# martende/findex

Measured on NVIDIA B200. Metric: fm_count_queries_per_s_len16_1GB_text, higher is better.
Workload: dtype u32

## Files before the change

### findex_b200/csrc/fmx_device.cuh

```cuda
#pragma once
#include <cstdint>
#include <cuda_runtime.h>

#include "../../include/fmgpu.h"

namespace fmx {

constexpr uint32_t kBitsPerBlock = 480;
constexpr int kCodeAbsent = 0xFF;

struct DevIndex {
    const uint4   *blocks;
    uint64_t       stride;
    const uint8_t *bwt;
    const uint32_t *C;
    const uint32_t *base;
    const uint8_t *code;
    const uint4   *mark;
    const uint32_t *samples;
    const uint4   *bm;
    uint32_t n, eof;
    int32_t  layout, levels;
    uint32_t z[8];
    int32_t  wmx_b, wmx_levels;
// ... 375 lines not shown
        if (stop) return false;
        base += G;
        if (base >= ix.dict_buckets) base = 0;
        first = false;
    }
    return false;
}

template <int G, bool STATS, bool BISECT, typename PatFn>
__device__ __forceinline__ bool dict_chain(const DevIndex &ix, const uint8_t *code, PatFn pat, int &i, uint32_t &sp, uint32_t &ep,
                                           uint32_t &touched, uint32_t &steps, int depth, bool top_known_missed = false) {
    const int Jc = ix.dict_Jc;
    const uint32_t bits = (uint32_t)ix.dict_bits;
    for (int t = (depth - ix.dict_D) / Jc + 1; t <= kDictMaxTiers && i >= 0 && depth < ix.dict_Dx; ++t) {
        const int j = (i + 1) < Jc ? (i + 1) : Jc;
        uint64_t syms = 0;
        bool ok = true;
        for (int k = 0; k < j; ++k) {
            const uint32_t c = pat(i - k), cd = code[c];
            ok = ok && (cd != (uint32_t)kCodeAbsent) && (c != 0);
            syms |= (uint64_t)cd << (bits * (uint32_t)k);
        }
        if (!ok) return true;
        uint32_t s, e;
        if (!top_known_missed && dict_probe<G, STATS>(ix, dict_chain_key(sp, j, t, syms), s, e, touched)) {
            sp = s; ep = e;
            i -= j;
            depth += j;
            if (STATS) steps += j;
            if (j < Jc) return true;
            continue;
        }
        if (!BISECT) return false;
        int lo = 0, hi = j - 1;
        uint32_t bs = 0, be = 0;
        const uint32_t psp = sp;
        while (lo < hi) {
            const int mid = (lo + hi + 1) >> 1;
            if (dict_probe<G, STATS>(ix, dict_chain_key(psp, mid, t, syms & ((1ull << (bits * (uint32_t)mid)) - 1ull)), s, e, touched)) { lo = mid; bs = s; be = e; }
            else hi = mid - 1;
        }
        if (lo > 0) { sp = bs; ep = be; i -= lo; if (STATS) steps += lo; }
        return true;
    }
    return true;
}

struct CtxQuery {
    unsigned long long qlo, qhi, mlo, mhi;
    uint32_t sh;
    bool zero, absent;
};
template <typename PatFn>
__device__ __forceinline__ CtxQuery ctx_query(const DevIndex &ix, const SharedTables &tb, PatFn pat, int j, int o) {
    CtxQuery q;
    const uint32_t bits = (uint32_t)ix.isat_bits;
    q.qlo = 0; q.qhi = 0;
    q.sh = (uint32_t)(ix.ctx_J - j) * bits;
    const uint32_t nb = (uint32_t)j * bits;
    q.mlo = nb >= 64 ? ~0ull : ((1ull << nb) - 1ull);
    q.mhi = nb <= 64 ? 0ull : ((1ull << (nb - 64)) - 1ull);
    q.zero = false; q.absent = false;
    if (ix.ctx_raw) {
        uint32_t w0, w1, w2;
        pat.bytes12(o, w0, w1, w2);
        q.qlo = ((unsigned long long)w1 << 32) | w0;
        q.qhi = w2;
        const unsigned long long l = q.qlo | ~q.mlo, h = (q.qhi & q.mhi) | ~q.mhi;
        q.zero = (((l - 0x0101010101010101ull) & ~l) | ((h - 0x0101010101010101ull) & ~h)) & 0x8080808080808080ull;
    } else {
        for (int k = 0; k < j; ++k) {
            const uint32_t pc = pat(o + k), cd = tb.code[pc];
            q.zero = q.zero || (pc == 0);
            q.absent = q.absent || (cd == (uint32_t)kCodeAbsent);
            const unsigned long long v = (unsigned long long)((cd + 1u) & ((1u << bits) - 1u));
            const uint32_t ob = (uint32_t)k * bits;
            if (ob < 64) { q.qlo |= v << ob; if (ob + bits > 64) q.qhi |= v >> (64 - ob); }
            else q.qhi |= v << (ob - 64);
        }
    }
    return q;
}
__device__ __forceinline__ bool ctx_match(const CtxQuery &q, const uint4 &b) {
    const unsigned long long elo = ((unsigned long long)b.z << 32) | b.y, ehi = b.w;
    unsigned long long lo, hi;
    if (q.sh == 0) { lo = elo; hi = ehi; }
    else if (q.sh < 64) { lo = (elo >> q.sh) | (ehi << (64 - q.sh)); hi = ehi >> q.sh; }
    else { lo = ehi >> (q.sh - 64); hi = 0; }
    return (((lo ^ q.qlo) & q.mlo) | ((hi ^ q.qhi) & q.mhi)) == 0ull;
}

constexpr uint32_t kKmerGroup = 8, kKmerWide = 0xFFu, kKmerInlineRows = 3;

template <int G, bool STATS, typename PatFn>
__device__ __forceinline__ void kmer_group(const DevIndex &ix, const SharedTables &tb, PatFn pat, bool fetch, uint32_t idx, int &i,
                                           uint32_t &sp, uint32_t &ep, uint32_t &touched, uint32_t &steps, uint32_t &pre_from,
                                           uint32_t &pre_best, uint32_t &pre_cnt) {
    const uint4 *blk = reinterpret_cast<const uint4 *>(ix.kmer) + (uint64_t)(idx / kKmerGroup) * 4;
    uint4 q0, q1, q2, q3;
    if constexpr (G == 1) {
        const uint32_t odd = threadIdx.x & 1u;
        const unsigned long long mine = reinterpret_cast<unsigned long long>(blk);
        const unsigned long long pe = __shfl_sync(0xFFFFFFFFu, mine, (threadIdx.x & 31u) & ~1u);
        const unsigned long long po = __shfl_sync(0xFFFFFFFFu, mine, (threadIdx.x & 31u) | 1u);
        const bool fe = __shfl_sync(0xFFFFFFFFu, fetch, (threadIdx.x & 31u) & ~1u), fo = __shfl_sync(0xFFFFFFFFu, fetch, (threadIdx.x & 31u) | 1u);
        uint4 x0 = make_uint4(0, 0, 0, 0), x1 = x0, y0 = x0, y1 = x0;
        if (fe) ldg256(reinterpret_cast<const uint4 *>(pe) + 2 * odd, x0, x1);
        if (fo) ldg256(reinterpret_cast<const uint4 *>(po) + 2 * odd, y0, y1);
        uint4 s0 = odd ? x0 : y0, s1 = odd ? x1 : y1;
        s0.x = __shfl_xor_sync(0xFFFFFFFFu, s0.x, 1); s0.y = __shfl_xor_sync(0xFFFFFFFFu, s0.y, 1);
        s0.z = __shfl_xor_sync(0xFFFFFFFFu, s0.z, 1); s0.w = __shfl_xor_sync(0xFFFFFFFFu, s0.w, 1);
        s1.x = __shfl_xor_sync(0xFFFFFFFFu, s1.x, 1); s1.y = __shfl_xor_sync(0xFFFFFFFFu, s1.y, 1);
        s1.z = __shfl_xor_sync(0xFFFFFFFFu, s1.z, 1); s1.w = __shfl_xor_sync(0xFFFFFFFFu, s1.w, 1);
        if (odd) { q0 = s0; q1 = s1; q2 = y0; q3 = y1; } else { q0 = x0; q1 = x1; q2 = s0; q3 = s1; }
    } else {
        if (!fetch) return;
        ldg256(blk, q0, q1);
        ldg256(blk + 2, q2, q3);
    }
    if (!fetch) return;
    const uint32_t e = idx % kKmerGroup, kind = q0.w >> 24, base = q0.x;
    uint32_t lo, hi;
    if (kind != kKmerWide) {
        const unsigned long long ends = ((unsigned long long)q0.z << 32) | q0.y;
        hi = base + (uint32_t)((ends >> (8 * e)) & 0xFFu);
        lo = base + (e ? (uint32_t)((ends >> (8 * e - 8)) & 0xFFu) : 0u);
    } else {
        auto end_of = [&](uint32_t k) {
            return k < 4 ? (k < 2 ? (k == 0 ? q1.x : q1.y) : (k == 2 ? q1.z : q1.w)) : (k < 6 ? (k == 4 ? q2.x : q2.y) : (k == 6 ? q2.z : q2.w));
        };
        hi = end_of(e);
        lo = (e ? end_of(e - 1) : base) + (((e < 4 ? q3.x : q3.y) >> (8 * (e & 3))) & 0xFFu);
    }
    if (lo < hi) { sp = lo; ep = hi; } else { sp = 0; ep = 0; }
    if (STATS) { touched += 1; steps += ix.kmer_k; }
    if (kind == kKmerWide || kind == 0 || ix.ctx == nullptr || sp >= ep || i < 0) return;
    const int rem = i + 1;
    const uint32_t rows = ep - sp;
    const int t = rem <= kCtxPlanMax ? (int)tb.plan[rem] : kCtxHops - 1;
    const uint32_t need = rem <= kCtxPlanMax ? (uint32_t)tb.plan[128 + rem] : (uint32_t)(rem / ix.ctx_J + 3);
    if (t != kCtxHops - 1 || rows > kCtxMaxRows || !(rows == 1u || rows * need <= (uint32_t)rem)) return;
    const int j = ix.ctx_J;
    const CtxQuery q = ctx_query(ix, tb, pat, j, rem - j);
    if (q.zero) return;
    uint32_t best = 0xFFFFFFFFu, cnt = 0;
#pragma unroll
    for (uint32_t k = 0; k < kKmerInlineRows; ++k) {
        const uint4 &pl = k == 0 ? q1 : k == 1 ? q2 : q3;
        if (k < kind && base + k >= sp && base + k < ep && !q.absent && ctx_match(q, pl)) { best = pl.x < best ? pl.x : best; ++cnt; }
    }
    if (ep <= base + kind) {
        if (cnt) { sp = best; ep = best + cnt; } else { sp = 0; ep = 0; }
        i -= j;
        if (STATS) steps += j;
    } else {
        const int lane = (G == 1) ? 0 : (threadIdx.x & (G - 1));
        pre_from = base + kind;
        pre_best = best;
        pre_cnt = lane == 0 ? cnt : 0u;
    }
}

constexpr int kSearchFresh = 0, kSearchTopMissed = 1, kSearchResume = 2, kSearchChainMissed = 3;
template <int G, int LAYOUT, bool STATS, typename PatFn>
__device__ __forceinline__ void search_pattern(const DevIndex &ix, const SharedTables &tb, PatFn pat, int len, bool active,
                                               uint32_t &sp, uint32_t &ep, uint32_t &touched, uint32_t &steps,
                                               int mode = kSearchFresh, uint32_t rsp = 0, uint32_t rep = 0, int rconsumed = 0) {
    const int lane = (G == 1) ? 0 : (threadIdx.x & (G - 1));
    const uint32_t gmask = group_mask<G>();
    sp = 0;
    ep = active ? ix.n : 0u;
    int i = len - 1;
    bool noshort = (ix.isat == nullptr);
    uint32_t pre_from = 0, pre_best = 0xFFFFFFFFu, pre_cnt = 0;
    bool kfetch = false;
    uint32_t kidx = 0;
    if (active && (mode == kSearchResume || mode == kSearchChainMissed)) {
        sp = rsp; ep = rep;
        i -= rconsumed;
        if (mode == kSearchChainMissed) dict_chain<G, STATS, true>(ix, tb.code, pat, i, sp, ep, touched, steps, rconsumed, true);
    } else if (active && i >= 0) {
        bool done = false;
        if (ix.dict != nullptr && len > ix.kmer_k) {
            const int K = ix.kmer_k;
            const uint32_t bits = (uint32_t)ix.dict_bits;
            int hi = len < ix.dict_D ? len : ix.dict_D;
            uint64_t full = 0;
            bool ok = true;
            for (int j = 0; j < hi; ++j) {
                const uint32_t c = pat(len - 1 - j), code = tb.code[c];
                ok = ok && (code != (uint32_t)kCodeAbsent) && (c != 0);
                full |= (uint64_t)code << (bits * (uint32_t)j);
            }
            if (ok) {
                int lo = K, d = hi;
                uint32_t bsp = 0, bep = 0;
                if (mode == kSearchTopMissed) { --hi; d = (lo + hi + 1) >> 1; }
                while (lo < hi) {
                    uint32_t s, e;
                    if (dict_probe<G, STATS>(ix, dict_key(full, d, bits), s, e, touched)) { lo = d; bsp = s; bep = e; }
                    else hi = d - 1;
                    d = (lo + hi + 1) >> 1;
                }
                if (lo > K) {
                    sp = bsp; ep = bep;
                    i -= lo;
                    done = true;
                    if (STATS) steps += lo;
                    if (lo == ix.dict_D && ix.dict_Dx > ix.dict_D) dict_chain<G, STATS, true>(ix, tb.code, pat, i, sp, ep, touched, steps, lo);
                }
            }
        }
        if (!done && ix.kmer != nullptr && len >= ix.kmer_k) {
            const int K = ix.kmer_k;
            uint32_t idx = 0;
            bool ok = true;
            for (int j = 0; j < K; ++j) {
                const uint32_t c = pat(ix.kmer_rows ? len - K + j : len - 1 - j), code = tb.code[c];
                ok = ok && (code != (uint32_t)kCodeAbsent) && (c != 0);
                idx = idx * ix.kmer_sigma + code;
            }
            if (ok) {
                i -= K;
                done = true;
                if (ix.kmer_rows) { kfetch = true; kidx = idx; }
                else {
                    const uint2 v = ldg64(ix.kmer + idx);
                    sp = v.x; ep = v.y;
                    if (STATS) { touched += 1; steps += K; }
                }
            }
        }
        if (!done) {
            const uint32_t c = pat(i);
            sp = tb.C[c];
            ep = tb.C[c + 1];
            --i;
            if (STATS) ++steps;
        }
    }
    if (ix.kmer != nullptr && ix.kmer_rows) kmer_group<G, STATS>(ix, tb, pat, kfetch, kidx, i, sp, ep, touched, steps, pre_from, pre_best, pre_cnt);
    bool noctx = (ix.ctx == nullptr && ix.ctx8 == nullptr);
    for (;;) {
        const bool go = (i >= 0) && (sp < ep);
        if (go) {
            bool stepped = false;
            const int rem = i + 1;
            if (!noctx && ix.ctx8 != nullptr && (ep - sp) <= kCtxMaxRows && rem >= ix.ctx8_J) {
                const int J = ix.ctx8_J, o = rem - J;
                uint32_t q = 0;
                bool zero = false, absent = false;
                for (int k = 0; k < J; ++k) {
                    const uint32_t pc = pat(o + k), cd = tb.code[pc];
                    zero = zero || (pc == 0);
                    absent = absent || (cd == (uint32_t)kCodeAbsent);
                    q |= (cd & 3u) << (2 * k);
                }
                if (zero) noctx = true;
                else {
                    uint32_t best = 0xFFFFFFFFu, cnt = 0;
                    if (!absent) {
                        for (uint32_t r = sp + (uint32_t)lane; r < ep; r += G) {
                            const uint2 e = ldg64(ix.ctx8 + r);
                            if (e.y == q && e.x != 0xFFFFFFFFu) { best = e.x < best ? e.x : best; ++cnt; }
                        }
                    }
                    if (STATS && lane == 0) { touched += absent ? 0u : ep - sp; steps += J; }
                    if (G >= 2) { best = min(best, __shfl_xor_sync(gmask, best, 1)); cnt += __shfl_xor_sync(gmask, cnt, 1); }
                    if (G >= 4) { best = min(best, __shfl_xor_sync(gmask, best, 2)); cnt += __shfl_xor_sync(gmask, cnt, 2); }
                    if (cnt) { sp = best; ep = best + cnt; } else { sp = 0; ep = 0; }
                    i -= J;
                    stepped = true;
                }
            }
            if (!stepped && !noctx && ix.ctx != nullptr && (ep - sp) <= kCtxMaxRows) {
                const uint32_t rows = ep - sp;
                const int t = rem <= kCtxPlanMax ? (int)tb.plan[rem] : kCtxHops - 1;
                const uint32_t need = rem <= kCtxPlanMax ? (uint32_t)tb.plan[128 + rem] : (uint32_t)(rem / ix.ctx_J + 3);
                if (rows == 1u || rows * need <= (uint32_t)rem) {
                    const int j = (int)tb.hops[t];
                    const CtxQuery q = ctx_query(ix, tb, pat, j, rem - j);
                    if (q.zero) noctx = true;
                    else {
                        const uint32_t from = sp > pre_from ? sp : pre_from;
                        uint32_t best = pre_best, cnt = pre_cnt;
                        if (!q.absent) {
                            for (uint32_t r = from + (uint32_t)lane; r < ep; r += G) {
                                uint4 a, b;
                                ldg256(ix.ctx + (uint64_t)r * 2, a, b);
                                if (ctx_match(q, b)) {
                                    const uint32_t row = t == 0 ? a.x : t == 1 ? a.y : t == 2 ? a.z : t == 3 ? a.w : b.x;
                                    best = row < best ? row : best;
                                    ++cnt;
                                }
                            }
                        }
                        pre_from = 0; pre_best = 0xFFFFFFFFu; pre_cnt = 0;
                        if (STATS && lane == 0) { touched += q.absent ? 0u : ep - from; steps += j; }
                        if (G >= 2) { best = min(best, __shfl_xor_sync(gmask, best, 1)); cnt += __shfl_xor_sync(gmask, cnt, 1); }
                        if (G >= 4) { best = min(best, __shfl_xor_sync(gmask, best, 2)); cnt += __shfl_xor_sync(gmask, cnt, 2); }
                        if (cnt) { sp = best; ep = best + cnt; } else { sp = 0; ep = 0; }
                        i -= j;
                        stepped = true;
                    }
                }
            }
            if (!stepped && !noshort && (ep - sp) == 1u && i >= 2 && i < ix.isat_syms) {
                const uint32_t q = ldg32(ix.sa + sp);
                const bool fits = q >= (uint32_t)rem;
                const uint32_t b0 = fits ? q - (uint32_t)rem : 0u;
                const uint4 e = ldg128(ix.isat + b0);
                const uint32_t bits = (uint32_t)ix.isat_bits, fmask = (1u << bits) - 1u;
                bool eq = fits, zero = false;
                for (int k = lane; k < rem; k += G) {
                    const uint32_t pc = pat(k);
                    const uint32_t o = (uint32_t)k * bits, w = o >> 5;
                    const uint32_t lo = w == 0 ? e.y : w == 1 ? e.z : e.w, hi = w == 0 ? e.z : w == 1 ? e.w : 0u;
                    const uint32_t sym = __funnelshift_r(lo, hi, o & 31u) & fmask;
                    zero = zero || (pc == 0);
                    eq = eq && (sym == (uint32_t)tb.code[pc] + 1u);
                }
                if (G > 1) { eq = __all_sync(gmask, eq); zero = __any_sync(gmask, zero); }
                if (zero) noshort = true;
                else {
                    if (eq) { sp = e.x; ep = e.x + 1; } else { sp = 0; ep = 0; }
                    i = -1;
                    stepped = true;
                    if (STATS) { touched += 2; steps += rem; }
                }
            }
            if (!stepped) {
                backward_step<G, LAYOUT, STATS>(ix, tb, pat(i), sp, ep, touched);
                --i;
                if (STATS) ++steps;
// ... 36 lines not shown
```

### findex_b200/csrc/fmx_kernels.cu

```cuda
#include "fmx_kernels.cuh"

#include <algorithm>

namespace fmx {

template <int G, int LAYOUT, bool STATS, typename OutT, int MINB = (LAYOUT == FMX_LAYOUT_WMX ? 5 : (G == 1) ? 6 : 8)>
__global__ void __launch_bounds__(kThreads, MINB)
count_fixed_kernel(const __grid_constant__ DevIndex ix, const uint8_t *__restrict__ pat, int len, long long m,
                   OutT *__restrict__ sp_out, OutT *__restrict__ ep_out, unsigned long long *stats, const __grid_constant__ PeerSinks sinks) {
    __shared__ SharedTables tb;
    extern __shared__ __align__(16) uint8_t spat[];
    constexpr int QPB = kThreads / G;
    load_tables(tb, ix);

    const long long q0 = (long long)blockIdx.x * QPB;
    const int nq = (int)((m - q0) < (long long)QPB ? (m - q0) : (long long)QPB);
    {
        const uint8_t *src = pat + q0 * len;
        const int nbytes = nq * len;
        if ((reinterpret_cast<uintptr_t>(src) & 15) == 0) {
            const int nvec = nbytes >> 4;
            for (int i = threadIdx.x; i < nvec; i += kThreads)
                reinterpret_cast<uint4 *>(spat)[i] = ldg128(reinterpret_cast<const uint4 *>(src) + i);
            for (int i = (nvec << 4) + threadIdx.x; i < nbytes; i += kThreads) spat[i] = src[i];
        } else {
            for (int i = threadIdx.x; i < nbytes; i += kThreads) spat[i] = src[i];
        }
    }
    __syncthreads();

    const int g = threadIdx.x / G;
    const bool active = g < nq;
    uint32_t sp, ep, touched = 0, steps = 0;
    search_pattern<G, LAYOUT, STATS>(ix, tb, SmemPattern{spat + g * len, len, (len & 3) == 0}, len, active, sp, ep, touched, steps);
    const bool hit = sp < ep;
    const uint32_t cnt = hit ? ep - sp : 0u;
    if (active && (threadIdx.x % G) == 0) {
        sp_out[q0 + g] = hit ? (OutT)sp : (OutT)0;
        ep_out[q0 + g] = hit ? (OutT)ep : (OutT)0;
        if (sinks.n == 1) sinks.p[0][sinks.offset + q0 + g] = cnt;
    }
    if (sinks.n > 1) {
        __shared__ __align__(16) uint32_t scnt[kThreads];
        if ((threadIdx.x % G) == 0) scnt[g] = active ? cnt : 0u;
        __syncthreads();
        const long long base = sinks.offset + q0;
        if (nq == QPB && (base & 3) == 0) {
            constexpr int V = QPB / 4;
            for (int w = threadIdx.x; w < sinks.n * V; w += kThreads) {
                const int j = w / V, k = w - j * V;
                reinterpret_cast<uint4 *>(sinks.p[j] + base)[k] = reinterpret_cast<const uint4 *>(scnt)[k];
            }
        } else {
            for (int w = threadIdx.x; w < sinks.n * nq; w += kThreads) {
                const int j = w / nq, k = w - j * nq;
                sinks.p[j][base + k] = scnt[k];
            }
        }
    }
    if (STATS) {
        if ((threadIdx.x % G) != 0) { touched = 0; steps = 0; }
        for (int o = 16; o; o >>= 1) {
            touched += __shfl_xor_sync(0xFFFFFFFFu, touched, o);
            steps += __shfl_xor_sync(0xFFFFFFFFu, steps, o);
        }
        if ((threadIdx.x & 31) == 0) { atomicAdd(&stats[0], (unsigned long long)touched); atomicAdd(&stats[1], (unsigned long long)steps); }
    }
}

template <int G, int LAYOUT, typename OutT>
__global__ void __launch_bounds__(kThreads)
count_fixed_gmem_kernel(const __grid_constant__ DevIndex ix, const uint8_t *__restrict__ pat, int len, long long m, OutT *__restrict__ sp_out,
                        OutT *__restrict__ ep_out, const __grid_constant__ PeerSinks sinks) {
    __shared__ SharedTables tb;
    load_tables(tb, ix);
    __syncthreads();
    constexpr int QPB = kThreads / G;
    const long long q = (long long)blockIdx.x * QPB + threadIdx.x / G;
    const bool active = q < m;
    uint32_t sp, ep, touched = 0, steps = 0;
    search_pattern<G, LAYOUT, false>(ix, tb, GlobalPattern{pat + (active ? q : 0) * len, len}, len, active, sp, ep, touched, steps);
    if (active && (threadIdx.x % G) == 0) {
        const bool hit = sp < ep;
        sp_out[q] = hit ? (OutT)sp : (OutT)0;
        ep_out[q] = hit ? (OutT)ep : (OutT)0;
        for (int j = 0; j < sinks.n; ++j) sinks.p[j][sinks.offset + q] = hit ? ep - sp : 0u;
    }
}

constexpr uint32_t kListModeShift = 30, kListIdMask = (1u << kListModeShift) - 1u;

template <typename OutT>
__global__ void __launch_bounds__(kThreads)
count_dict_first_kernel(const __grid_constant__ DevIndex ix, const uint8_t *__restrict__ pat, int len, long long m, OutT *__restrict__ sp_out,
                        OutT *__restrict__ ep_out, uint2 *__restrict__ list, unsigned long long *__restrict__ list_count,
                        const __grid_constant__ PeerSinks sinks) {
    __shared__ uint8_t scode[256];
    extern __shared__ __align__(16) uint8_t spat[];
    for (int i = threadIdx.x; i < 256; i += kThreads) scode[i] = ix.code[i];
    const int d0 = len < ix.dict_D ? len : ix.dict_D;
    const long long q0 = (long long)blockIdx.x * kThreads;
    const int nq = (int)((m - q0) < (long long)kThreads ? (m - q0) : (long long)kThreads);
    {
        const uint8_t *src = pat + q0 * len;
        const int nbytes = nq * len;
        if ((reinterpret_cast<uintptr_t>(src) & 15) == 0) {
            const int nvec = nbytes >> 4;
            for (int i = threadIdx.x; i < nvec; i += kThreads)
                reinterpret_cast<uint4 *>(spat)[i] = ldg128(reinterpret_cast<const uint4 *>(src) + i);
            for (int i = (nvec << 4) + threadIdx.x; i < nbytes; i += kThreads) spat[i] = src[i];
        } else {
            for (int i = threadIdx.x; i < nbytes; i += kThreads) spat[i] = src[i];
        }
    }
    __syncthreads();
    const bool active = (int)threadIdx.x < nq;
    const long long q = q0 + threadIdx.x;
    uint32_t entry = 0xFFFFFFFFu, consumed = 0;
    if (active) {
        const uint8_t *p = spat + (size_t)threadIdx.x * len;
        const uint32_t bits = (uint32_t)ix.dict_bits;
        uint64_t full = 0;
        bool ok = true;
        for (int j = 0; j < d0; ++j) {
            const uint32_t c = p[len - 1 - j], code = scode[c];
            ok = ok && (code != (uint32_t)kCodeAbsent) && (c != 0);
            full |= (uint64_t)code << (bits * (uint32_t)j);
        }
        entry = (uint32_t)threadIdx.x | ((uint32_t)kSearchFresh << kListModeShift);
        if (ok) {
            uint32_t s = 0, e = 0, touched = 0;
            if (dict_probe<1, false>(ix, dict_key(full, d0, bits), s, e, touched)) {
                int i = len - 1 - d0;
                bool chain_open = true;
                if (i >= 0 && ix.dict_Dx > ix.dict_D) {
                    uint32_t steps = 0;
                    chain_open = dict_chain<1, false, false>(ix, scode, SmemPattern{p, len, false}, i, s, e, touched, steps, d0);
                }
                consumed = (uint32_t)(len - 1 - i);
                sp_out[q] = (OutT)s;
                ep_out[q] = (OutT)e;
                if (i < 0) {
                    entry = 0xFFFFFFFFu;
                    for (int j = 0; j < sinks.n; ++j) sinks.p[j][sinks.offset + q] = e - s;
                } else entry = (uint32_t)threadIdx.x | ((uint32_t)(chain_open ? kSearchResume : kSearchChainMissed) << kListModeShift);
            } else entry = (uint32_t)threadIdx.x | ((uint32_t)kSearchTopMissed << kListModeShift);
        }
    }
    __shared__ uint32_t wcount[kThreads / 32];
    __shared__ unsigned long long cta_base;
    const uint32_t need = __ballot_sync(0xFFFFFFFFu, entry != 0xFFFFFFFFu);
    const int lane = threadIdx.x & 31, warp = threadIdx.x >> 5;
    if (lane == 0) wcount[warp] = (uint32_t)__popc(need);
    __syncthreads();
    if (threadIdx.x == 0) {
        uint32_t total = 0;
        for (int w = 0; w < kThreads / 32; ++w) { const uint32_t c = wcount[w]; wcount[w] = total; total += c; }
        cta_base = total ? atomicAdd(list_count, (unsigned long long)total) : 0ull;
    }
    __syncthreads();
    if (entry != 0xFFFFFFFFu) {
        const uint32_t mode = entry >> kListModeShift;
        list[cta_base + wcount[warp] + __popc(need & ((1u << lane) - 1u))] = make_uint2((uint32_t)(q0 + (entry & kListIdMask)) | (mode << kListModeShift), consumed);
    }
}

template <int G, int LAYOUT, typename OutT>
__global__ void __launch_bounds__(kThreads)
count_list_kernel(const __grid_constant__ DevIndex ix, const uint8_t *__restrict__ pat, int len, OutT *__restrict__ sp_out, OutT *__restrict__ ep_out,
                  const uint2 *__restrict__ list, const unsigned long long *__restrict__ list_count, const __grid_constant__ PeerSinks sinks) {
    __shared__ SharedTables tb;
    extern __shared__ __align__(16) uint8_t spat[];
    constexpr int QPB = kThreads / G;
    const unsigned long long count = *list_count;
    if ((unsigned long long)blockIdx.x * QPB >= count) return;
    load_tables(tb, ix);
    const int g = threadIdx.x / G, lane = threadIdx.x % G;
    const int stride = (len + 3) & ~3;
    {
        const unsigned long long t = (unsigned long long)blockIdx.x * QPB + g;
        const bool active = t < count;
        const uint2 le = active ? list[t] : make_uint2(0u, 0u);
        const uint32_t entry = le.x;
        const long long q = (long long)(entry & kListIdMask);
        const int mode = (int)(entry >> kListModeShift);
        __syncthreads();
        if (active) {
            const uint8_t *src = pat + q * len;
            uint8_t *dst = spat + (size_t)g * stride;
            if ((len & 3) == 0 && (reinterpret_cast<uintptr_t>(src) & 3) == 0)
                for (int w = lane; w < (len >> 2); w += G) reinterpret_cast<uint32_t *>(dst)[w] = __ldg(reinterpret_cast<const uint32_t *>(src) + w);
            else
                for (int b = lane; b < len; b += G) dst[b] = __ldg(src + b);
        }
        __syncthreads();
        uint32_t rsp = 0, rep = 0;
        if (active && (mode == kSearchResume || mode == kSearchChainMissed)) { rsp = (uint32_t)sp_out[q]; rep = (uint32_t)ep_out[q]; }
        uint32_t sp, ep, touched = 0, steps = 0;
        search_pattern<G, LAYOUT, false>(ix, tb, SmemPattern{spat + (size_t)g * stride, len, true}, len, active, sp, ep, touched, steps, mode, rsp, rep, (int)le.y);
        if (active && (threadIdx.x % G) == 0) {
            const bool hit = sp < ep;
            sp_out[q] = hit ? (OutT)sp : (OutT)0;
            ep_out[q] = hit ? (OutT)ep : (OutT)0;
            for (int j = 0; j < sinks.n; ++j) sinks.p[j][sinks.offset + q] = hit ? ep - sp : 0u;
        }
    }
}

template <int G, int LAYOUT>
__global__ void __launch_bounds__(kThreads)
count_var_kernel(const __grid_constant__ DevIndex ix, const uint8_t *__restrict__ pat, const long long *__restrict__ off,
                 long long m, long long *__restrict__ sp_out, long long *__restrict__ ep_out) {
    __shared__ SharedTables tb;
    load_tables(tb, ix);
    __syncthreads();
    constexpr int QPB = kThreads / G;
    const long long q = (long long)blockIdx.x * QPB + threadIdx.x / G;
    const bool active = q < m;
    long long lo = 0, hi = 0;
    if (active) { lo = off[q]; hi = off[q + 1]; }
    uint32_t sp, ep, touched = 0, steps = 0;
    search_pattern<G, LAYOUT, false>(ix, tb, GlobalPattern{pat + lo, (int)(hi - lo)}, (int)(hi - lo), active, sp, ep, touched, steps);
    if (active && (threadIdx.x % G) == 0) {
        const bool hit = sp < ep;
        sp_out[q] = hit ? (long long)sp : 0;
        ep_out[q] = hit ? (long long)ep : 0;
    }
}

template <int G, int LAYOUT>
__global__ void __launch_bounds__(kThreads)
occ_kernel(const __grid_constant__ DevIndex ix, const uint8_t *__restrict__ c, const long long *__restrict__ key, long long m,
           long long *__restrict__ out) {
    __shared__ SharedTables tb;
    load_tables(tb, ix);
    __syncthreads();
    const long long q = (long long)blockIdx.x * (kThreads / G) + threadIdx.x / G;
    if (q >= m) return;
    long long k = key[q] + 1;
    k = k < 0 ? 0 : (k > (long long)ix.n ? (long long)ix.n : k);
    const uint32_t cc = c[q];
    const uint32_t v = lf_value<G, LAYOUT>(ix, tb, cc, (uint32_t)k);
    if ((threadIdx.x % G) == 0) out[q] = (long long)(v - tb.C[cc]);
}

template <int G, int LAYOUT>
__global__ void __launch_bounds__(kThreads)
prev_range_kernel(const __grid_constant__ DevIndex ix, const long long *__restrict__ sp, const long long *__restrict__ ep,
                  const uint8_t *__restrict__ c, long long m, long long *__restrict__ sp1, long long *__restrict__ ep1) {
    __shared__ SharedTables tb;
    load_tables(tb, ix);
    __syncthreads();
// ... 216 lines not shown
              unsigned long long *sink) {
    const long long gid = ((long long)blockIdx.x * kThreads + threadIdx.x) / LANES;
    const int lane = threadIdx.x % LANES;
    if (gid >= gathers) return;
    unsigned long long x = (unsigned long long)gid * 0x9E3779B97F4A7C15ull + seed;
    uint32_t acc = 0;
    for (int s = 0; s < chain; ++s) {
        x ^= x >> 33; x *= 0xFF51AFD7ED558CCDull; x ^= x >> 33; x *= 0xC4CEB9FE1A85EC53ull; x ^= x >> 33;
        const unsigned long long unit = __umul64hi(x, n_units);
        const uint4 *p = base + unit * (LANES * VEC) + lane * VEC;
        uint32_t v = 0;
#pragma unroll
        for (int i = 0; i < VEC; ++i) { const uint4 q = ldg128(p + i); v ^= q.x ^ q.y ^ q.z ^ q.w; }
        if (LANES > 1) {
            const uint32_t mask = ((LANES == 32) ? 0xFFFFFFFFu : ((1u << LANES) - 1u)) << ((threadIdx.x & 31) & ~(LANES - 1));
            for (int o = 1; o < LANES; o <<= 1) v ^= __shfl_xor_sync(mask, v, o);
        }
        acc ^= v;
        x += v;
    }
    if (acc == 0x12345678u && lane == 0) atomicAdd(sink, 1ull);
}

#define FMX_DISPATCH(cfg, CALL)                                                                      \
    do {                                                                                             \
        if ((cfg).layout == FMX_LAYOUT_PLANES) {                                                     \
            if ((cfg).lanes == 1) { CALL(1, FMX_LAYOUT_PLANES); }                                    \
            else if ((cfg).lanes == 2) { CALL(2, FMX_LAYOUT_PLANES); }                               \
            else { CALL(4, FMX_LAYOUT_PLANES); }                                                     \
        } else if ((cfg).layout == FMX_LAYOUT_WMX) {                                                 \
            if ((cfg).lanes == 1) { CALL(1, FMX_LAYOUT_WMX); }                                       \
            else if ((cfg).lanes == 2) { CALL(2, FMX_LAYOUT_WMX); }                                  \
            else { CALL(4, FMX_LAYOUT_WMX); }                                                        \
        } else {                                                                                     \
            if ((cfg).lanes == 1) { CALL(1, FMX_LAYOUT_WM); }                                        \
            else if ((cfg).lanes == 2) { CALL(2, FMX_LAYOUT_WM); }                                   \
            else { CALL(4, FMX_LAYOUT_WM); }                                                         \
        }                                                                                            \
    } while (0)

static inline unsigned grid_for(int64_t items, int lanes) {
    const int64_t per = kThreads / lanes;
    return (unsigned)((items + per - 1) / per);
}

cudaError_t launch_count_fixed(const DevIndex &ix, LaunchCfg cfg, const uint8_t *d_pat, int len, int64_t m, void *d_sp,
                               void *d_ep, bool out64, unsigned long long *d_stats, cudaStream_t st, const PeerSinks *sinks_or_null) {
    if (m <= 0) return cudaSuccess;
    if (cfg.count_lanes) cfg.lanes = cfg.count_lanes;
    PeerSinks sinks{};
    if (sinks_or_null) sinks = *sinks_or_null;
    const size_t smem = (size_t)(kThreads / cfg.lanes) * (size_t)(len > 0 ? len : 1) + 16;
    const bool too_long = smem > 160 * 1024;
    if (ix.dict != nullptr && len > ix.kmer_k && len <= ix.dict_Dx && !d_stats && m < (1ll << kListModeShift) && (size_t)kThreads * (size_t)len <= 160 * 1024) {
        unsigned long long *cnt = nullptr;
        cudaError_t e = cudaMallocAsync(&cnt, 16 + (size_t)m * 8, st);
        if (e != cudaSuccess) return e;
        uint2 *list = reinterpret_cast<uint2 *>(cnt + 2);
        cudaMemsetAsync(cnt, 0, 8, st);
        const size_t smem1 = (size_t)kThreads * (size_t)len;
        const unsigned grid1 = grid_for(m, 1);
        if (out64) {
            auto k = count_dict_first_kernel<long long>;
            cudaFuncSetAttribute(k, cudaFuncAttributeMaxDynamicSharedMemorySize, (int)smem1);
            k<<<grid1, kThreads, smem1, st>>>(ix, d_pat, len, m, (long long *)d_sp, (long long *)d_ep, list, cnt, sinks);
        } else {
            auto k = count_dict_first_kernel<uint32_t>;
            cudaFuncSetAttribute(k, cudaFuncAttributeMaxDynamicSharedMemorySize, (int)smem1);
            k<<<grid1, kThreads, smem1, st>>>(ix, d_pat, len, m, (uint32_t *)d_sp, (uint32_t *)d_ep, list, cnt, sinks);
        }
        const unsigned grid2 = grid_for(m, cfg.lanes);
#define CALL2(G, LAY)                                                                                                  \
        {                                                                                                              \
            const size_t smem2 = (size_t)(kThreads / G) * (size_t)((len + 3) & ~3) + 16;                               \
            if (out64) count_list_kernel<G, LAY, long long><<<grid2, kThreads, smem2, st>>>(ix, d_pat, len, (long long *)d_sp, (long long *)d_ep, list, cnt, sinks); \
            else count_list_kernel<G, LAY, uint32_t><<<grid2, kThreads, smem2, st>>>(ix, d_pat, len, (uint32_t *)d_sp, (uint32_t *)d_ep, list, cnt, sinks); \
        }
        FMX_DISPATCH(cfg, CALL2);
#undef CALL2
        cudaFreeAsync(cnt, st);
        return cudaGetLastError();
    }
#define CALL(G, LAY)                                                                                                  \
    {                                                                                                                 \
        if (too_long && !d_stats) {                                                                                   \
            if (out64) count_fixed_gmem_kernel<G, LAY, long long><<<grid_for(m, G), kThreads, 0, st>>>(ix, d_pat, len, m, (long long *)d_sp, (long long *)d_ep, sinks); \
            else count_fixed_gmem_kernel<G, LAY, uint32_t><<<grid_for(m, G), kThreads, 0, st>>>(ix, d_pat, len, m, (uint32_t *)d_sp, (uint32_t *)d_ep, sinks); \
        } else if (too_long) {                                                                                        \
            return cudaErrorInvalidValue;                                                                             \
        } else if (d_stats) {                                                                                                \
            auto k = count_fixed_kernel<G, LAY, true, uint32_t>;                                                      \
            cudaFuncSetAttribute(k, cudaFuncAttributeMaxDynamicSharedMemorySize, (int)smem);                          \
            k<<<grid_for(m, G), kThreads, smem, st>>>(ix, d_pat, len, m, (uint32_t *)d_sp, (uint32_t *)d_ep, d_stats, sinks); \
        } else if (out64) {                                                                                           \
            auto k = count_fixed_kernel<G, LAY, false, long long>;                                                    \
            cudaFuncSetAttribute(k, cudaFuncAttributeMaxDynamicSharedMemorySize, (int)smem);                          \
            k<<<grid_for(m, G), kThreads, smem, st>>>(ix, d_pat, len, m, (long long *)d_sp, (long long *)d_ep, nullptr, sinks); \
        } else if (cfg.min_blocks >= 4 && cfg.min_blocks <= 8) {                      \
            auto k = cfg.min_blocks == 4 ? count_fixed_kernel<G, LAY, false, uint32_t, 4> : cfg.min_blocks == 5 ? count_fixed_kernel<G, LAY, false, uint32_t, 5> : \
                     cfg.min_blocks == 6 ? count_fixed_kernel<G, LAY, false, uint32_t, 6> : cfg.min_blocks == 7 ? count_fixed_kernel<G, LAY, false, uint32_t, 7> : \
                     count_fixed_kernel<G, LAY, false, uint32_t, 8>;                                                  \
            cudaFuncSetAttribute(k, cudaFuncAttributeMaxDynamicSharedMemorySize, (int)smem);                          \
            k<<<grid_for(m, G), kThreads, smem, st>>>(ix, d_pat, len, m, (uint32_t *)d_sp, (uint32_t *)d_ep, nullptr, sinks); \
        } else {                                                                                                      \
            auto k = count_fixed_kernel<G, LAY, false, uint32_t>;                                                     \
            cudaFuncSetAttribute(k, cudaFuncAttributeMaxDynamicSharedMemorySize, (int)smem);                          \
            k<<<grid_for(m, G), kThreads, smem, st>>>(ix, d_pat, len, m, (uint32_t *)d_sp, (uint32_t *)d_ep, nullptr, sinks); \
        }                                                                                                             \
    }
    FMX_DISPATCH(cfg, CALL);
#undef CALL
    return cudaGetLastError();
}

cudaError_t launch_count_var(const DevIndex &ix, LaunchCfg cfg, const uint8_t *d_pat, const int64_t *d_off, int64_t m,
                             int64_t *d_sp, int64_t *d_ep, cudaStream_t st) {
    if (m <= 0) return cudaSuccess;
    if (cfg.count_lanes) cfg.lanes = cfg.count_lanes;
#define CALL(G, LAY) count_var_kernel<G, LAY><<<grid_for(m, G), kThreads, 0, st>>>(ix, d_pat, (const long long *)d_off, m, (long long *)d_sp, (long long *)d_ep)
    FMX_DISPATCH(cfg, CALL);
#undef CALL
    return cudaGetLastError();
}

cudaError_t launch_occ(const DevIndex &ix, LaunchCfg cfg, const uint8_t *d_c, const int64_t *d_key, int64_t m, int64_t *d_out,
                       cudaStream_t st) {
    if (m <= 0) return cudaSuccess;
#define CALL(G, LAY) occ_kernel<G, LAY><<<grid_for(m, G), kThreads, 0, st>>>(ix, d_c, (const long long *)d_key, m, (long long *)d_out)
    FMX_DISPATCH(cfg, CALL);
#undef CALL
    return cudaGetLastError();
}
// ... 82 lines not shown
```

Baseline: 27.51 billion.

## Split k-mer plus context queries into a per-thread first pass and compacted list

Adds a group-split path for patterns whose length equals kmer_k plus ctx_J. A one-thread-per-query kernel resolves the k-mer block and inline context rows and writes final results directly. Unresolved queries go to a compacted list carrying resume state, and a second kernel finishes them with multiple rounds per block. This is meant to avoid running the whole grouped search on every query when most resolve cheaply, at the cost of an extra launch, an allocation and list traffic.

```diff
diff --git a/findex_b200/csrc/fmx_device.cuh b/findex_b200/csrc/fmx_device.cuh
--- a/findex_b200/csrc/fmx_device.cuh
+++ b/findex_b200/csrc/fmx_device.cuh
@@ -451,7 +451,7 @@
     bool zero, absent;
 };
 template <typename PatFn>
-__device__ __forceinline__ CtxQuery ctx_query(const DevIndex &ix, const SharedTables &tb, PatFn pat, int j, int o) {
+__device__ __forceinline__ CtxQuery ctx_query(const DevIndex &ix, const uint8_t *code, PatFn pat, int j, int o) {
     CtxQuery q;
     const uint32_t bits = (uint32_t)ix.isat_bits;
     q.qlo = 0; q.qhi = 0;
@@ -469,7 +469,7 @@
         q.zero = (((l - 0x0101010101010101ull) & ~l) | ((h - 0x0101010101010101ull) & ~h)) & 0x8080808080808080ull;
     } else {
         for (int k = 0; k < j; ++k) {
-            const uint32_t pc = pat(o + k), cd = tb.code[pc];
+            const uint32_t pc = pat(o + k), cd = code[pc];
             q.zero = q.zero || (pc == 0);
             q.absent = q.absent || (cd == (uint32_t)kCodeAbsent);
             const unsigned long long v = (unsigned long long)((cd + 1u) & ((1u << bits) - 1u));
@@ -491,12 +491,12 @@
 
 constexpr uint32_t kKmerGroup = 8, kKmerWide = 0xFFu, kKmerInlineRows = 3;
 
-template <int G, bool STATS, typename PatFn>
-__device__ __forceinline__ void kmer_group(const DevIndex &ix, const SharedTables &tb, PatFn pat, bool fetch, uint32_t idx, int &i,
-                                           uint32_t &sp, uint32_t &ep, uint32_t &touched, uint32_t &steps, uint32_t &pre_from,
-                                           uint32_t &pre_best, uint32_t &pre_cnt) {
+struct KmerBlock { uint4 q0, q1, q2, q3; };
+
+template <int G>
+__device__ __forceinline__ KmerBlock kmer_block_fetch(const DevIndex &ix, bool fetch, uint32_t idx) {
     const uint4 *blk = reinterpret_cast<const uint4 *>(ix.kmer) + (uint64_t)(idx / kKmerGroup) * 4;
-    uint4 q0, q1, q2, q3;
+    KmerBlock b;
     if constexpr (G == 1) {
         const uint32_t odd = threadIdx.x & 1u;
         const unsigned long long mine = reinterpret_cast<unsigned long long>(blk);
@@ -511,67 +511,85 @@
         s0.z = __shfl_xor_sync(0xFFFFFFFFu, s0.z, 1); s0.w = __shfl_xor_sync(0xFFFFFFFFu, s0.w, 1);
         s1.x = __shfl_xor_sync(0xFFFFFFFFu, s1.x, 1); s1.y = __shfl_xor_sync(0xFFFFFFFFu, s1.y, 1);
         s1.z = __shfl_xor_sync(0xFFFFFFFFu, s1.z, 1); s1.w = __shfl_xor_sync(0xFFFFFFFFu, s1.w, 1);
-        if (odd) { q0 = s0; q1 = s1; q2 = y0; q3 = y1; } else { q0 = x0; q1 = x1; q2 = s0; q3 = s1; }
+        if (odd) { b.q0 = s0; b.q1 = s1; b.q2 = y0; b.q3 = y1; } else { b.q0 = x0; b.q1 = x1; b.q2 = s0; b.q3 = s1; }
     } else {
-        if (!fetch) return;
-        ldg256(blk, q0, q1);
-        ldg256(blk + 2, q2, q3);
-    }
-    if (!fetch) return;
-    const uint32_t e = idx % kKmerGroup, kind = q0.w >> 24, base = q0.x;
+        b.q0 = b.q1 = b.q2 = b.q3 = make_uint4(0, 0, 0, 0);
+        if (fetch) { ldg256(blk, b.q0, b.q1); ldg256(blk + 2, b.q2, b.q3); }
+    }
+    return b;
+}
+
+template <typename PatFn>
+__device__ __forceinline__ void kmer_block_decode(const DevIndex &ix, const uint8_t *code, PatFn pat, const KmerBlock &b, uint32_t idx, int t,
+                                                  uint32_t need, bool lane0, int &i, uint32_t &sp, uint32_t &ep, uint32_t &pre_from,
+                                                  uint32_t &pre_best, uint32_t &pre_cnt) {
+    const uint32_t e = idx % kKmerGroup, kind = b.q0.w >> 24, base = b.q0.x;
     uint32_t lo, hi;
     if (kind != kKmerWide) {
-        const unsigned long long ends = ((unsigned long long)q0.z << 32) | q0.y;
+        const unsigned long long ends = ((unsigned long long)b.q0.z << 32) | b.q0.y;
         hi = base + (uint32_t)((ends >> (8 * e)) & 0xFFu);
         lo = base + (e ? (uint32_t)((ends >> (8 * e - 8)) & 0xFFu) : 0u);
     } else {
         auto end_of = [&](uint32_t k) {
-            return k < 4 ? (k < 2 ? (k == 0 ? q1.x : q1.y) : (k == 2 ? q1.z : q1.w)) : (k < 6 ? (k == 4 ? q2.x : q2.y) : (k == 6 ? q2.z : q2.w));
+            return k < 4 ? (k < 2 ? (k == 0 ? b.q1.x : b.q1.y) : (k == 2 ? b.q1.z : b.q1.w)) : (k < 6 ? (k == 4 ? b.q2.x : b.q2.y) : (k == 6 ? b.q2.z : b.q2.w));
         };
         hi = end_of(e);
-        lo = (e ? end_of(e - 1) : base) + (((e < 4 ? q3.x : q3.y) >> (8 * (e & 3))) & 0xFFu);
+        lo = (e ? end_of(e - 1) : base) + (((e < 4 ? b.q3.x : b.q3.y) >> (8 * (e & 3))) & 0xFFu);
     }
     if (lo < hi) { sp = lo; ep = hi; } else { sp = 0; ep = 0; }
-    if (STATS) { touched += 1; steps += ix.kmer_k; }
     if (kind == kKmerWide || kind == 0 || ix.ctx == nullptr || sp >= ep || i < 0) return;
     const int rem = i + 1;
     const uint32_t rows = ep - sp;
-    const int t = rem <= kCtxPlanMax ? (int)tb.plan[rem] : kCtxHops - 1;
-    const uint32_t need = rem <= kCtxPlanMax ? (uint32_t)tb.plan[128 + rem] : (uint32_t)(rem / ix.ctx_J + 3);
     if (t != kCtxHops - 1 || rows > kCtxMaxRows || !(rows == 1u || rows * need <= (uint32_t)rem)) return;
     const int j = ix.ctx_J;
-    const CtxQuery q = ctx_query(ix, tb, pat, j, rem - j);
+    const CtxQuery q = ctx_query(ix, code, pat, j, rem - j);
     if (q.zero) return;
     uint32_t best = 0xFFFFFFFFu, cnt = 0;
 #pragma unroll
     for (uint32_t k = 0; k < kKmerInlineRows; ++k) {
-        const uint4 &pl = k == 0 ? q1 : k == 1 ? q2 : q3;
+        const uint4 &pl = k == 0 ? b.q1 : k == 1 ? b.q2 : b.q3;
         if (k < kind && base + k >= sp && base + k < ep && !q.absent && ctx_match(q, pl)) { best = pl.x < best ? pl.x : best; ++cnt; }
     }
     if (ep <= base + kind) {
         if (cnt) { sp = best; ep = best + cnt; } else { sp = 0; ep = 0; }
         i -= j;
-        if (STATS) steps += j;
     } else {
-        const int lane = (G == 1) ? 0 : (threadIdx.x & (G - 1));
         pre_from = base + kind;
         pre_best = best;
-        pre_cnt = lane == 0 ? cnt : 0u;
-    }
+        pre_cnt = lane0 ? cnt : 0u;
+    }
+}
+
+template <int G, bool STATS, typename PatFn>
+__device__ __forceinline__ void kmer_group(const DevIndex &ix, const SharedTables &tb, PatFn pat, bool fetch, uint32_t idx, int &i,
+                                           uint32_t &sp, uint32_t &ep, uint32_t &touched, uint32_t &steps, uint32_t &pre_from,
+                                           uint32_t &pre_best, uint32_t &pre_cnt) {
+    const KmerBlock b = kmer_block_fetch<G>(ix, fetch, idx);
+    if (!fetch) return;
+    const int rem = i + 1, i0 = i;
+    int t = 0;
+    uint32_t need = 0;
+    if (ix.ctx != nullptr && rem > 0) {
+        t = rem <= kCtxPlanMax ? (int)tb.plan[rem] : kCtxHops - 1;
+        need = rem <= kCtxPlanMax ? (uint32_t)tb.plan[128 + rem] : (uint32_t)(rem / ix.ctx_J + 3);
+    }
+    kmer_block_decode(ix, tb.code, pat, b, idx, t, need, G == 1 || (threadIdx.x & (G - 1)) == 0, i, sp, ep, pre_from, pre_best, pre_cnt);
+    if (STATS) { touched += 1; steps += ix.kmer_k + (i0 - i); }
 }
 
 constexpr int kSearchFresh = 0, kSearchTopMissed = 1, kSearchResume = 2, kSearchChainMissed = 3;
 template <int G, int LAYOUT, bool STATS, typename PatFn>
 __device__ __forceinline__ void search_pattern(const DevIndex &ix, const SharedTables &tb, PatFn pat, int len, bool active,
                                                uint32_t &sp, uint32_t &ep, uint32_t &touched, uint32_t &steps,
-                                               int mode = kSearchFresh, uint32_t rsp = 0, uint32_t rep = 0, int rconsumed = 0) {
+                                               int mode = kSearchFresh, uint32_t rsp = 0, uint32_t rep = 0, int rconsumed = 0,
+                                               uint32_t rbest = 0xFFFFFFFFu, uint32_t rcnt = 0) {
     const int lane = (G == 1) ? 0 : (threadIdx.x & (G - 1));
     const uint32_t gmask = group_mask<G>();
     sp = 0;
     ep = active ? ix.n : 0u;
     int i = len - 1;
     bool noshort = (ix.isat == nullptr);
-    uint32_t pre_from = 0, pre_best = 0xFFFFFFFFu, pre_cnt = 0;
+    uint32_t pre_from = 0, pre_best = rbest, pre_cnt = lane == 0 ? rcnt : 0u;
     bool kfetch = false;
     uint32_t kidx = 0;
     if (active && (mode == kSearchResume || mode == kSearchChainMissed)) {
@@ -678,7 +696,7 @@
                 const uint32_t need = rem <= kCtxPlanMax ? (uint32_t)tb.plan[128 + rem] : (uint32_t)(rem / ix.ctx_J + 3);
                 if (rows == 1u || rows * need <= (uint32_t)rem) {
                     const int j = (int)tb.hops[t];
-                    const CtxQuery q = ctx_query(ix, tb, pat, j, rem - j);
+                    const CtxQuery q = ctx_query(ix, tb.code, pat, j, rem - j);
                     if (q.zero) noctx = true;
                     else {
                         const uint32_t from = sp > pre_from ? sp : pre_from;
diff --git a/findex_b200/csrc/fmx_kernels.cu b/findex_b200/csrc/fmx_kernels.cu
--- a/findex_b200/csrc/fmx_kernels.cu
+++ b/findex_b200/csrc/fmx_kernels.cu
@@ -3,6 +3,37 @@
 #include <algorithm>
 
 namespace fmx {
+
+__device__ __forceinline__ void stage_patterns(uint8_t *spat, const uint8_t *src, int nbytes) {
+    if ((reinterpret_cast<uintptr_t>(src) & 15) == 0) {
+        const int nvec = nbytes >> 4;
+        for (int i = threadIdx.x; i < nvec; i += kThreads)
+            reinterpret_cast<uint4 *>(spat)[i] = ldg128(reinterpret_cast<const uint4 *>(src) + i);
+        for (int i = (nvec << 4) + threadIdx.x; i < nbytes; i += kThreads) spat[i] = src[i];
+    } else {
+        for (int i = threadIdx.x; i < nbytes; i += kThreads) spat[i] = src[i];
+    }
+}
+
+template <int QPB>
+__device__ __forceinline__ void store_counts_to_sinks(const PeerSinks &sinks, long long q0, int nq, int g, bool store, uint32_t cnt) {
+    __shared__ __align__(16) uint32_t scnt[QPB];
+    if (store) scnt[g] = cnt;
+    __syncthreads();
+    const long long base = sinks.offset + q0;
+    if (nq == QPB && (base & 3) == 0) {
+        constexpr int V = QPB / 4;
+        for (int w = threadIdx.x; w < sinks.n * V; w += kThreads) {
+            const int j = w / V, k = w - j * V;
+            reinterpret_cast<uint4 *>(sinks.p[j] + base)[k] = reinterpret_cast<const uint4 *>(scnt)[k];
+        }
+    } else {
+        for (int w = threadIdx.x; w < sinks.n * nq; w += kThreads) {
+            const int j = w / nq, k = w - j * nq;
+            sinks.p[j][base + k] = scnt[k];
+        }
+    }
+}
 
 template <int G, int LAYOUT, bool STATS, typename OutT, int MINB = (LAYOUT == FMX_LAYOUT_WMX ? 5 : (G == 1) ? 6 : 8)>
 __global__ void __launch_bounds__(kThreads, MINB)
@@ -15,18 +46,7 @@
 
     const long long q0 = (long long)blockIdx.x * QPB;
     const int nq = (int)((m - q0) < (long long)QPB ? (m - q0) : (long long)QPB);
-    {
-        const uint8_t *src = pat + q0 * len;
-        const int nbytes = nq * len;
-        if ((reinterpret_cast<uintptr_t>(src) & 15) == 0) {
-            const int nvec = nbytes >> 4;
-            for (int i = threadIdx.x; i < nvec; i += kThreads)
-                reinterpret_cast<uint4 *>(spat)[i] = ldg128(reinterpret_cast<const uint4 *>(src) + i);
-            for (int i = (nvec << 4) + threadIdx.x; i < nbytes; i += kThreads) spat[i] = src[i];
-        } else {
-            for (int i = threadIdx.x; i < nbytes; i += kThreads) spat[i] = src[i];
-        }
-    }
+    stage_patterns(spat, pat + q0 * len, nq * len);
     __syncthreads();
 
     const int g = threadIdx.x / G;
@@ -40,24 +60,7 @@
         ep_out[q0 + g] = hit ? (OutT)ep : (OutT)0;
         if (sinks.n == 1) sinks.p[0][sinks.offset + q0 + g] = cnt;
     }
-    if (sinks.n > 1) {
-        __shared__ __align__(16) uint32_t scnt[kThreads];
-        if ((threadIdx.x % G) == 0) scnt[g] = active ? cnt : 0u;
-        __syncthreads();
-        const long long base = sinks.offset + q0;
-        if (nq == QPB && (base & 3) == 0) {
-            constexpr int V = QPB / 4;
-            for (int w = threadIdx.x; w < sinks.n * V; w += kThreads) {
-                const int j = w / V, k = w - j * V;
-                reinterpret_cast<uint4 *>(sinks.p[j] + base)[k] = reinterpret_cast<const uint4 *>(scnt)[k];
-            }
-        } else {
-            for (int w = threadIdx.x; w < sinks.n * nq; w += kThreads) {
-                const int j = w / nq, k = w - j * nq;
-                sinks.p[j][base + k] = scnt[k];
-            }
-        }
-    }
+    if (sinks.n > 1) store_counts_to_sinks<QPB>(sinks, q0, nq, g, (threadIdx.x % G) == 0, active ? cnt : 0u);
     if (STATS) {
         if ((threadIdx.x % G) != 0) { touched = 0; steps = 0; }
         for (int o = 16; o; o >>= 1) {
@@ -90,6 +93,22 @@
 
 constexpr uint32_t kListModeShift = 30, kListIdMask = (1u << kListModeShift) - 1u;
 
+__device__ __forceinline__ unsigned long long list_slot(bool listed, unsigned long long *list_count) {
+    __shared__ uint32_t wcount[kThreads / 32];
+    __shared__ unsigned long long cta_base;
+    const uint32_t need = __ballot_sync(0xFFFFFFFFu, listed);
+    const int lane = threadIdx.x & 31, warp = threadIdx.x >> 5;
+    if (lane == 0) wcount[warp] = (uint32_t)__popc(need);
+    __syncthreads();
+    if (threadIdx.x == 0) {
+        uint32_t total = 0;
+        for (int w = 0; w < kThreads / 32; ++w) { const uint32_t c = wcount[w]; wcount[w] = total; total += c; }
+        cta_base = total ? atomicAdd(list_count, (unsigned long long)total) : 0ull;
+    }
+    __syncthreads();
+    return cta_base + wcount[warp] + __popc(need & ((1u << lane) - 1u));
+}
+
 template <typename OutT>
 __global__ void __launch_bounds__(kThreads)
 count_dict_first_kernel(const __grid_constant__ DevIndex ix, const uint8_t *__restrict__ pat, int len, long long m, OutT *__restrict__ sp_out,
@@ -101,18 +120,7 @@
     const int d0 = len < ix.dict_D ? len : ix.dict_D;
     const long long q0 = (long long)blockIdx.x * kThreads;
     const int nq = (int)((m - q0) < (long long)kThreads ? (m - q0) : (long long)kThreads);
-    {
-        const uint8_t *src = pat + q0 * len;
-        const int nbytes = nq * len;
-        if ((reinterpret_cast<uintptr_t>(src) & 15) == 0) {
-            const int nvec = nbytes >> 4;
-            for (int i = threadIdx.x; i < nvec; i += kThreads)
-                reinterpret_cast<uint4 *>(spat)[i] = ldg128(reinterpret_cast<const uint4 *>(src) + i);
-            for (int i = (nvec << 4) + threadIdx.x; i < nbytes; i += kThreads) spat[i] = src[i];
-        } else {
-            for (int i = threadIdx.x; i < nbytes; i += kThreads) spat[i] = src[i];
-        }
-    }
+    stage_patterns(spat, pat + q0 * len, nq * len);
     __syncthreads();
     const bool active = (int)threadIdx.x < nq;
     const long long q = q0 + threadIdx.x;
@@ -147,43 +155,90 @@
             } else entry = (uint32_t)threadIdx.x | ((uint32_t)kSearchTopMissed << kListModeShift);
         }
     }
-    __shared__ uint32_t wcount[kThreads / 32];
-    __shared__ unsigned long long cta_base;
-    const uint32_t need = __ballot_sync(0xFFFFFFFFu, entry != 0xFFFFFFFFu);
-    const int lane = threadIdx.x & 31, warp = threadIdx.x >> 5;
-    if (lane == 0) wcount[warp] = (uint32_t)__popc(need);
-    __syncthreads();
-    if (threadIdx.x == 0) {
-        uint32_t total = 0;
-        for (int w = 0; w < kThreads / 32; ++w) { const uint32_t c = wcount[w]; wcount[w] = total; total += c; }
-        cta_base = total ? atomicAdd(list_count, (unsigned long long)total) : 0ull;
-    }
-    __syncthreads();
+    const unsigned long long slot = list_slot(entry != 0xFFFFFFFFu, list_count);
     if (entry != 0xFFFFFFFFu) {
         const uint32_t mode = entry >> kListModeShift;
-        list[cta_base + wcount[warp] + __popc(need & ((1u << lane) - 1u))] = make_uint2((uint32_t)(q0 + (entry & kListIdMask)) | (mode << kListModeShift), consumed);
-    }
-}
-
-template <int G, int LAYOUT, typename OutT>
+        list[slot] = make_uint2((uint32_t)(q0 + (entry & kListIdMask)) | (mode << kListModeShift), consumed);
+    }
+}
+
+template <typename OutT>
+__global__ void __launch_bounds__(kThreads, 8)
+count_group_first_kernel(const __grid_constant__ DevIndex ix, const uint8_t *__restrict__ pat, int len, long long m, OutT *__restrict__ sp_out,
+                         OutT *__restrict__ ep_out, uint4 *__restrict__ list, unsigned long long *__restrict__ list_count,
+                         const __grid_constant__ PeerSinks sinks) {
+    __shared__ uint8_t scode[256];
+    extern __shared__ __align__(16) uint8_t spat[];
+    const long long q0 = (long long)blockIdx.x * kThreads;
+    const int nq = (int)((m - q0) < (long long)kThreads ? (m - q0) : (long long)kThreads);
+    stage_patterns(spat, pat + q0 * len, nq * len);
+    for (int i = threadIdx.x; i < 256; i += kThreads) scode[i] = ix.code[i];
+    const int K = ix.kmer_k, rem = len - K;
+    const int t = (int)__ldg(ix.ctx_plan + rem);
+    const uint32_t need = (uint32_t)__ldg(ix.ctx_plan + 128 + rem);
+    __syncthreads();
+    const bool active = (int)threadIdx.x < nq;
+    const SmemPattern p{spat + (size_t)threadIdx.x * len, len, (len & 3) == 0};
+    uint32_t idx = 0;
+    bool ok = active;
+    for (int j = 0; j < K; ++j) {
+        const uint32_t c = p(rem + j), code = scode[c];
+        ok = ok && (code != (uint32_t)kCodeAbsent) && (c != 0);
+        idx = idx * ix.kmer_sigma + code;
+    }
+    const KmerBlock b = kmer_block_fetch<1>(ix, ok, idx);
+    int i = rem - 1;
+    uint32_t sp = 0, ep = 0, pre_from = 0, pre_best = 0xFFFFFFFFu, pre_cnt = 0;
+    if (ok) kmer_block_decode(ix, scode, p, b, idx, t, need, true, i, sp, ep, pre_from, pre_best, pre_cnt);
+    const bool listed = active && (!ok || (sp < ep && i >= 0));
+    const uint32_t cnt = (active && !listed && sp < ep) ? ep - sp : 0u;
+    const long long q = q0 + threadIdx.x;
+    if (active && !listed) {
+        sp_out[q] = cnt ? (OutT)sp : (OutT)0;
+        ep_out[q] = cnt ? (OutT)ep : (OutT)0;
+        if (sinks.n == 1) sinks.p[0][sinks.offset + q] = cnt;
+    }
+    if (sinks.n > 1) store_counts_to_sinks<kThreads>(sinks, q0, nq, threadIdx.x, true, cnt);
+    const unsigned long long slot = list_slot(listed, list_count);
+    if (listed) {
+        const uint32_t from = sp > pre_from ? sp : pre_from;
+        list[slot] = make_uint4((uint32_t)q | (pre_cnt << kListModeShift), ok ? from : 0u, ok ? ep : 0u, pre_best);
+    }
+}
+
+constexpr int kGroupListRounds = 4;
+template <int G, int LAYOUT, typename OutT, typename Entry>
 __global__ void __launch_bounds__(kThreads)
 count_list_kernel(const __grid_constant__ DevIndex ix, const uint8_t *__restrict__ pat, int len, OutT *__restrict__ sp_out, OutT *__restrict__ ep_out,
-                  const uint2 *__restrict__ list, const unsigned long long *__restrict__ list_count, const __grid_constant__ PeerSinks sinks) {
+                  const Entry *__restrict__ list, const unsigned long long *__restrict__ list_count, const __grid_constant__ PeerSinks sinks,
+                  int rounds) {
+    constexpr bool kGroup = sizeof(Entry) == 16;
     __shared__ SharedTables tb;
     extern __shared__ __align__(16) uint8_t spat[];
     constexpr int QPB = kThreads / G;
     const unsigned long long count = *list_count;
-    if ((unsigned long long)blockIdx.x * QPB >= count) return;
+    const unsigned long long first = (unsigned long long)blockIdx.x * rounds * QPB;
+    if (first >= count) return;
     load_tables(tb, ix);
     const int g = threadIdx.x / G, lane = threadIdx.x % G;
     const int stride = (len + 3) & ~3;
-    {
-        const unsigned long long t = (unsigned long long)blockIdx.x * QPB + g;
+    for (int r = 0; r < rounds && first + (unsigned long long)r * QPB < count; ++r) {
+        const unsigned long long t = first + (unsigned long long)r * QPB + g;
         const bool active = t < count;
-        const uint2 le = active ? list[t] : make_uint2(0u, 0u);
+        Entry le{};
+        if (active) le = list[t];
         const uint32_t entry = le.x;
         const long long q = (long long)(entry & kListIdMask);
-        const int mode = (int)(entry >> kListModeShift);
+        int mode, consumed;
+        uint32_t rsp = 0, rep = 0, rbest = 0xFFFFFFFFu, rcnt = 0;
+        if constexpr (kGroup) {
+            rsp = le.y; rep = le.z; rbest = le.w; rcnt = entry >> kListModeShift;
+            mode = rsp < rep ? kSearchResume : kSearchFresh;
+            consumed = ix.kmer_k;
+        } else {
+            mode = (int)(entry >> kListModeShift);
+            consumed = (int)le.y;
+        }
         __syncthreads();
         if (active) {
             const uint8_t *src = pat + q * len;
@@ -194,10 +249,10 @@
                 for (int b = lane; b < len; b += G) dst[b] = __ldg(src + b);
         }
         __syncthreads();
-        uint32_t rsp = 0, rep = 0;
-        if (active && (mode == kSearchResume || mode == kSearchChainMissed)) { rsp = (uint32_t)sp_out[q]; rep = (uint32_t)ep_out[q]; }
+        if (!kGroup && active && (mode == kSearchResume || mode == kSearchChainMissed)) { rsp = (uint32_t)sp_out[q]; rep = (uint32_t)ep_out[q]; }
         uint32_t sp, ep, touched = 0, steps = 0;
-        search_pattern<G, LAYOUT, false>(ix, tb, SmemPattern{spat + (size_t)g * stride, len, true}, len, active, sp, ep, touched, steps, mode, rsp, rep, (int)le.y);
+        search_pattern<G, LAYOUT, false>(ix, tb, SmemPattern{spat + (size_t)g * stride, len, true}, len, active, sp, ep, touched, steps, mode, rsp, rep,
+                                         consumed, rbest, rcnt);
         if (active && (threadIdx.x % G) == 0) {
             const bool hit = sp < ep;
             sp_out[q] = hit ? (OutT)sp : (OutT)0;
@@ -520,32 +575,40 @@
     if (sinks_or_null) sinks = *sinks_or_null;
     const size_t smem = (size_t)(kThreads / cfg.lanes) * (size_t)(len > 0 ? len : 1) + 16;
     const bool too_long = smem > 160 * 1024;
-    if (ix.dict != nullptr && len > ix.kmer_k && len <= ix.dict_Dx && !d_stats && m < (1ll << kListModeShift) && (size_t)kThreads * (size_t)len <= 160 * 1024) {
+    const bool list_ok = !d_stats && m < (1ll << kListModeShift) && (size_t)kThreads * (size_t)len <= 160 * 1024;
+    const bool dict_split = list_ok && ix.dict != nullptr && len > ix.kmer_k && len <= ix.dict_Dx;
+    const bool group_split = list_ok && !dict_split && ix.kmer != nullptr && ix.kmer_rows > 0 && ix.ctx != nullptr && ix.ctx8 == nullptr &&
+                             ix.dict == nullptr && len == ix.kmer_k + ix.ctx_J && len - ix.kmer_k <= kCtxPlanMax;
+    if (dict_split || group_split) {
+        const size_t esize = dict_split ? sizeof(uint2) : sizeof(uint4);
         unsigned long long *cnt = nullptr;
-        cudaError_t e = cudaMallocAsync(&cnt, 16 + (size_t)m * 8, st);
+        cudaError_t e = cudaMallocAsync(&cnt, 16 + (size_t)m * esize, st);
         if (e != cudaSuccess) return e;
-        uint2 *list = reinterpret_cast<uint2 *>(cnt + 2);
+        void *list = cnt + 2;
         cudaMemsetAsync(cnt, 0, 8, st);
-        const size_t smem1 = (size_t)kThreads * (size_t)len;
+        const size_t smem1 = (size_t)kThreads * (size_t)len + (group_split ? 16 : 0);
         const unsigned grid1 = grid_for(m, 1);
-        if (out64) {
-            auto k = count_dict_first_kernel<long long>;
-            cudaFuncSetAttribute(k, cudaFuncAttributeMaxDynamicSharedMemorySize, (int)smem1);
-            k<<<grid1, kThreads, smem1, st>>>(ix, d_pat, len, m, (long long *)d_sp, (long long *)d_ep, list, cnt, sinks);
-        } else {
-            auto k = count_dict_first_kernel<uint32_t>;
-            cudaFuncSetAttribute(k, cudaFuncAttributeMaxDynamicSharedMemorySize, (int)smem1);
-            k<<<grid1, kThreads, smem1, st>>>(ix, d_pat, len, m, (uint32_t *)d_sp, (uint32_t *)d_ep, list, cnt, sinks);
-        }
-        const unsigned grid2 = grid_for(m, cfg.lanes);
-#define CALL2(G, LAY)                                                                                                  \
+#define CALL1(KERNEL, OUT, ENTRY)                                                                                      \
+        {                                                                                                              \
+            auto k = KERNEL<OUT>;                                                                                      \
+            cudaFuncSetAttribute(k, cudaFuncAttributeMaxDynamicSharedMemorySize, (int)smem1);                          \
+            k<<<grid1, kThreads, smem1, st>>>(ix, d_pat, len, m, (OUT *)d_sp, (OUT *)d_ep, (ENTRY *)list, cnt, sinks);  \
+        }
+        if (dict_split) { if (out64) CALL1(count_dict_first_kernel, long long, uint2) else CALL1(count_dict_first_kernel, uint32_t, uint2) }
+        else { if (out64) CALL1(count_group_first_kernel, long long, uint4) else CALL1(count_group_first_kernel, uint32_t, uint4) }
+#undef CALL1
+        const int rounds = dict_split ? 1 : kGroupListRounds;
+        const unsigned grid2 = (unsigned)((m + (int64_t)(kThreads / cfg.lanes) * rounds - 1) / ((int64_t)(kThreads / cfg.lanes) * rounds));
+#define CALL2E(G, LAY, ENTRY)                                                                                          \
         {                                                                                                              \
             const size_t smem2 = (size_t)(kThreads / G) * (size_t)((len + 3) & ~3) + 16;                               \
-            if (out64) count_list_kernel<G, LAY, long long><<<grid2, kThreads, smem2, st>>>(ix, d_pat, len, (long long *)d_sp, (long long *)d_ep, list, cnt, sinks); \
-            else count_list_kernel<G, LAY, uint32_t><<<grid2, kThreads, smem2, st>>>(ix, d_pat, len, (uint32_t *)d_sp, (uint32_t *)d_ep, list, cnt, sinks); \
-        }
+            if (out64) count_list_kernel<G, LAY, long long, ENTRY><<<grid2, kThreads, smem2, st>>>(ix, d_pat, len, (long long *)d_sp, (long long *)d_ep, (const ENTRY *)list, cnt, sinks, rounds); \
+            else count_list_kernel<G, LAY, uint32_t, ENTRY><<<grid2, kThreads, smem2, st>>>(ix, d_pat, len, (uint32_t *)d_sp, (uint32_t *)d_ep, (const ENTRY *)list, cnt, sinks, rounds); \
+        }
+#define CALL2(G, LAY) { if (dict_split) CALL2E(G, LAY, uint2) else CALL2E(G, LAY, uint4) }
         FMX_DISPATCH(cfg, CALL2);
 #undef CALL2
+#undef CALL2E
         cudaFreeAsync(cnt, st);
         return cudaGetLastError();
     }
```

New measurement: 30.97 billion (median of 6 runs). +12.6%, better.
